# Dahan-Wang/Rethinking-Flow-and-Diffusion-Bridge-Models-for-Speech-Enhancement

Hardware: NVIDIA B200
Metric: enhanced audio-sec/sec (5-step SB bridge, ncsnpp_v2) (higher is better)
Workload: dtype fp16

## Files before the change

### rethinking-flow-and-diffusion-bridge-models-for-speech-enhancement_b200/csrc/conv_igemm.cu

```cuda
#include <cuda.h>
#include <mutex>
#include <type_traits>
#include "common.cuh"
#include "tc05.cuh"

namespace fdbm {
int make_act_tile_map(CUtensorMap* map, const op_t* ptr, int B, int T, int F, int C, int box_f, int box_t);
namespace {

using namespace tc05;

constexpr int MT = 2;
constexpr int TILE_T = 16, TILE_F = 8;
constexpr int HALO_T = TILE_T + 2, HALO_F = TILE_F + 2;
constexpr int A_TILE_BYTES = HALO_T * HALO_F * 128;
constexpr int A_TILE_STRIDE = 23552;
constexpr int A_STAGES = 3;
constexpr int B_STAGES = 3;
constexpr int BN = 128;
constexpr int B_TILE_BYTES = BN * 128;
constexpr int A_SBO = HALO_F * 128;
constexpr int NUM_THREADS = 512;
constexpr int EPI_GROUPS = 2;
constexpr int MAX_SEG = 3;
constexpr int MAX_KB = 16;
constexpr int A_TILE1_BYTES = TILE_T * TILE_F * 128;
constexpr int PIPE_REGS = 56, EPI_REGS = 168, XFORM_REGS = 120;
constexpr int STAGE_BYTES = EPI_GROUPS * 4 * 32 * 32 * 4;
constexpr int STAT_SLOTS = 2;
constexpr int STAT_BYTES = EPI_GROUPS * 4 * BN * 8;
constexpr int B_STAGES_NARROW = B_STAGES * B_TILE_BYTES / (16 * 128);
constexpr int SMEM_BYTES = A_STAGES * MT * A_TILE_STRIDE + B_STAGES * B_TILE_BYTES + STAGE_BYTES + STAT_BYTES + 512;

struct SegParams {
  int taps, norm, act, tab_stride;
  int halo;
  const float2* tab;
};

struct ConvParams {
  int B, T, F, Cout;
  int n_seg, n_kb;
  SegParams seg[MAX_SEG];
  uint32_t ksched[MAX_KB];
  int tiles_t, tiles_f, n_mtiles, n_nblocks, n_items;
  uint32_t mg_tiles_t, mg_tiles_f, mg_nblocks;
  int bn;
  int side_ring, n_main, side_gap, n_steps;
  const float* bias;
  const float* bias_b;
  int bias_b_stride;
  const float* residual;
  const op_t* residual_h16;
  float scale;
  float* out_f32;
  op_t* out_h16;
  double* sums;
  float* pyr_out;
  const float* pyr_prev;
  int pyr_C;
  const float* comb_pyr;
  const float* comb_w;
  const float* comb_b;
  int comb_C;
};

struct TileCoord { int b, t0, f0; bool valid; };

__device__ __forceinline__ int fast_div(int n, int d, uint32_t mg) { return d == 1 ? n : static_cast<int>(__umulhi(static_cast<uint32_t>(n), mg)); }
__device__ __forceinline__ int item_tile(const ConvParams& p, int item) { return fast_div(item, p.n_nblocks, p.mg_nblocks); }
__device__ __forceinline__ int item_nblk(const ConvParams& p, int item) { return item - item_tile(p, item) * p.n_nblocks; }

__device__ __forceinline__ TileCoord decode_tile(const ConvParams& p, int mi) {
  TileCoord c;
  c.valid = mi < p.n_mtiles;
  const int rest = fast_div(mi, p.tiles_t, p.mg_tiles_t);
  const int tt = mi - rest * p.tiles_t;
  c.t0 = tt * TILE_T;
  c.b = fast_div(rest, p.tiles_f, p.mg_tiles_f);
  c.f0 = (rest - c.b * p.tiles_f) * TILE_F;
  return c;
}

template <typename F>
__device__ __forceinline__ void walk_steps(const ConvParams& p, F&& f) {
  const int n_side = p.n_kb - p.n_main;
  int sd = 0, cnt = 0;
  for (int m = 0; m < p.n_main; ++m) {
    const int ntaps = p.seg[p.ksched[m] & 15].taps;
    for (int tap = 0; tap < ntaps; ++tap) {
      f(false, m, tap, ntaps);
      if (++cnt == p.side_gap && sd < n_side) { f(true, p.n_main + sd, 0, 1); ++sd; cnt = 0; }
    }
  }
  for (; sd < n_side; ++sd) f(true, p.n_main + sd, 0, 1);
}

template <bool COMB, bool RES16>
__global__ void __launch_bounds__(NUM_THREADS, 1)
conv_igemm_kernel(const __grid_constant__ CUtensorMap map_a0, const __grid_constant__ CUtensorMap map_a1,
                  const __grid_constant__ CUtensorMap map_a2, const __grid_constant__ CUtensorMap map_b,
                  const ConvParams p) {
  extern __shared__ __align__(1024) uint8_t smem_raw[];
  uint8_t* smem = smem_raw;
  if (smem_u32(smem_raw) & 1023u) __trap();
  uint8_t* sA = smem;
  uint8_t* sB = smem + A_STAGES * MT * A_TILE_STRIDE;
  uint8_t* s_stage = sB + B_STAGES * B_TILE_BYTES;
  uint8_t* s_stat = s_stage + STAGE_BYTES;
  uint64_t* bars = reinterpret_cast<uint64_t*>(s_stage + STAGE_BYTES + STAT_BYTES);
  uint64_t* a_full = bars;
  uint64_t* a_empty = a_full + A_STAGES;
  uint64_t* b_full = a_empty + A_STAGES;
  uint64_t* b_empty = b_full + B_STAGES_NARROW;
  uint64_t* acc_full = b_empty + B_STAGES_NARROW;
  const int b_stages = p.bn == 16 ? B_STAGES_NARROW : B_STAGES;
  const int b_stride = p.bn * 128;
  uint64_t* acc_empty = acc_full + 2;
  uint64_t* a_ready = acc_empty + 2;
  uint64_t* side_full = a_ready + A_STAGES;
  uint64_t* side_empty = side_full + 1;
  uint32_t* tmem_slot = reinterpret_cast<uint32_t*>(side_empty + 1);
  static_assert((3 * A_STAGES + 2 * B_STAGES_NARROW + 4 + 2) * 8 + 4 <= 512, "barrier region");
  const int a_stages = p.side_ring ? A_STAGES - 1 : A_STAGES;
  const int n_main = p.side_ring ? p.n_main : p.n_kb;
// ... 14 lines not shown
    if (p.n_seg > 1) tma_prefetch_desc(&map_a1);
    if (p.n_seg > 2) tma_prefetch_desc(&map_a2);
  }
  if (warp == 3) {
    tmem_alloc(tmem_slot, 512);
    tmem_relinquish();
  }
  fence_before_sync();
  __syncthreads();
  fence_after_sync();
  const uint32_t tmem_base = *tmem_slot;
  asm volatile("griddepcontrol.wait;" ::: "memory");
  asm volatile("griddepcontrol.launch_dependents;" ::: "memory");

  if (warp < 4) {
  reg_dec<PIPE_REGS>();
  if (warp == 0) {
    if (lane == 0) {
      uint32_t stage = 0, phase = 0;
      for (int item = blockIdx.x; item < p.n_items; item += gridDim.x) {
        const int ct = item_tile(p, item);
        TileCoord tc[MT];
        int n_valid = 0;
        for (int j = 0; j < MT; ++j) { tc[j] = decode_tile(p, ct * MT + j); n_valid += tc[j].valid; }
        for (int i = 0; i < n_main; ++i) {
          const uint32_t e = p.ksched[i];
          const int sgi = e & 15, c0 = ((e >> 4) & 0xFFF) * 64;
          const int halo = p.seg[sgi].halo;
          mbar_wait_relaxed<256>(a_empty + stage, phase ^ 1);
          mbar_expect_tx(a_full + stage, n_valid * (halo ? A_TILE_BYTES : A_TILE1_BYTES));
          const CUtensorMap* map = sgi == 0 ? &map_a0 : (sgi == 1 ? &map_a1 : &map_a2);
          for (int j = 0; j < MT; ++j) {
            if (!tc[j].valid) continue;
            tma_load_4d(sA + (stage * MT + j) * A_TILE_STRIDE, map, a_full + stage, c0, tc[j].f0 - halo, tc[j].t0 - halo,
                        tc[j].b);
          }
          if (++stage == a_stages) { stage = 0; phase ^= 1; }
        }
      }
    }
  } else if (warp == 3) {
    if (lane == 0 && p.side_ring) {
      uint32_t phase = 0;
      for (int item = blockIdx.x; item < p.n_items; item += gridDim.x) {
        const int ct = item_tile(p, item);
        TileCoord tc[MT];
        int n_valid = 0;
        for (int j = 0; j < MT; ++j) { tc[j] = decode_tile(p, ct * MT + j); n_valid += tc[j].valid; }
        for (int i = n_main; i < n_kb; ++i) {
          const uint32_t e = p.ksched[i];
          const int sgi = e & 15, c0 = ((e >> 4) & 0xFFF) * 64;
          mbar_wait_relaxed<128>(side_empty, phase ^ 1);
          mbar_expect_tx(side_full, n_valid * A_TILE1_BYTES);
          const CUtensorMap* map = sgi == 0 ? &map_a0 : (sgi == 1 ? &map_a1 : &map_a2);
          for (int j = 0; j < MT; ++j) {
            if (!tc[j].valid) continue;
            tma_load_4d(sA + ((A_STAGES - 1) * MT + j) * A_TILE_STRIDE, map, side_full, c0, tc[j].f0, tc[j].t0, tc[j].b);
          }
          phase ^= 1;
        }
      }
    }
  } else if (warp == 1) {
    if (lane == 0) {
      uint32_t stage = 0, phase = 0;
      for (int item = blockIdx.x; item < p.n_items; item += gridDim.x) {
        const int n0 = item_nblk(p, item) * BN;
        if (p.side_ring) {
          walk_steps(p, [&](bool, int idx, int tap, int) {
            const int kt = static_cast<int>(p.ksched[idx] >> 16) + tap;
            mbar_wait_relaxed<128>(b_empty + stage, phase ^ 1);
            mbar_expect_tx(b_full + stage, b_stride);
            tma_load_2d(sB + stage * b_stride, &map_b, b_full + stage, 0, kt * p.Cout + n0);
            if (++stage == b_stages) { stage = 0; phase ^= 1; }
          });
          continue;
        }
        for (int i = 0; i < n_kb; ++i) {
          const uint32_t e = p.ksched[i];
          const int ntaps = p.seg[e & 15].taps;
          int kt = e >> 16;
          for (int tap = 0; tap < ntaps; ++tap, ++kt) {
            mbar_wait_relaxed<128>(b_empty + stage, phase ^ 1);
            mbar_expect_tx(b_full + stage, b_stride);
            tma_load_2d(sB + stage * b_stride, &map_b, b_full + stage, 0, kt * p.Cout + n0);
            if (++stage == b_stages) { stage = 0; phase ^= 1; }
          }
        }
      }
    }
  } else if (warp == 2) {
    const uint32_t idesc = make_idesc_f16(128, p.bn, kOperandIsBf16);
    const uint64_t a_hi9 = make_desc_sw128(0, A_SBO) & 0xFFFFFFFF00000000ull;
    const uint64_t a_hi1 = make_desc_sw128(0, TILE_F * 128) & 0xFFFFFFFF00000000ull;
    const uint64_t b_hi = make_desc_sw128(0, 1024) & 0xFFFFFFFF00000000ull;
    const uint32_t lo_const = 1u << 16;
    const uint32_t sA_lo = (smem_u32(sA) & 0x3FFFF) >> 4, sB_lo = (smem_u32(sB) & 0x3FFFF) >> 4;
    uint32_t sa = 0, pa = 0, sb = 0, pb = 0, as = 0, pacc = 0, ps = 0;
    for (int item = blockIdx.x; item < p.n_items; item += gridDim.x) {
      const int ct = item_tile(p, item);
      const bool valid1 = (ct * MT + 1) < p.n_mtiles;
      mbar_wait(acc_empty + as, pacc ^ 1);
      fence_after_sync();
      uint32_t accumulate = 0;
      const uint32_t d0 = tmem_base + (as * MT) * BN, d1 = d0 + BN;
      if (p.side_ring) {
        int step = 0;
        walk_steps(p, [&](bool side, int idx, int tap, int ntaps) {
          const SegParams& sg = p.seg[p.ksched[idx] & 15];
          uint32_t a_base0, a_off = 0;
          if (side) {
            mbar_wait(side_full, ps);
            fence_after_sync();
            a_base0 = sA_lo + (((A_STAGES - 1) * MT) * A_TILE_STRIDE >> 4);
          } else {
            if (tap == 0) {
              mbar_wait(sg.norm ? a_ready + sa : a_full + sa, pa);
              fence_after_sync();
            }
            a_base0 = sA_lo + ((sa * MT) * A_TILE_STRIDE >> 4);
            const int df = ntaps == 9 ? tap / 3 : sg.halo, dt = ntaps == 9 ? tap - 3 * (tap / 3) : sg.halo;
            a_off = ((dt * HALO_F + df) * 128) >> 4;
          }
          const uint64_t a_hi = sg.halo ? a_hi9 : a_hi1;
          mbar_wait(b_full + sb, pb);
          fence_after_sync();
          const uint32_t b_lo = (sB_lo + (sb * b_stride >> 4)) | lo_const;
          const uint32_t a_lo0 = (a_base0 + a_off) | lo_const, a_lo1 = (a_base0 + (A_TILE_STRIDE >> 4) + a_off) | lo_const;
          const bool last_tap = tap == ntaps - 1;
          if (elect_one()) {
#pragma unroll
            for (int k = 0; k < 4; ++k)
              mma_f16(d0, a_hi | (a_lo0 + 2 * k), b_hi | (b_lo + 2 * k), idesc, k == 0 ? accumulate : 1u);
            if (valid1) {
#pragma unroll
              for (int k = 0; k < 4; ++k)
                mma_f16(d1, a_hi | (a_lo1 + 2 * k), b_hi | (b_lo + 2 * k), idesc, k == 0 ? accumulate : 1u);
            }
            mma_commit(b_empty + sb);
            if (side) mma_commit(side_empty);
            else if (last_tap) mma_commit(a_empty + sa);
            if (step == p.n_steps - 1) mma_commit(acc_full + as);
          }
          __syncwarp();
          accumulate = 1;
          ++step;
          if (++sb == b_stages) { sb = 0; pb ^= 1; }
          if (side) ps ^= 1;
          else if (last_tap && ++sa == a_stages) { sa = 0; pa ^= 1; }
        });
        if (++as == 2) { as = 0; pacc ^= 1; }
        continue;
      }
      for (int i = 0; i < n_kb; ++i) {
        const SegParams& sg = p.seg[p.ksched[i] & 15];
        const int ntaps = sg.taps;
        const uint64_t a_hi = sg.halo ? a_hi9 : a_hi1;
        mbar_wait(sg.norm ? a_ready + sa : a_full + sa, pa);
        fence_after_sync();
        const uint32_t a_base0 = sA_lo + ((sa * MT) * A_TILE_STRIDE >> 4), a_base1 = a_base0 + (A_TILE_STRIDE >> 4);
        int df = ntaps == 9 ? 0 : sg.halo, dt = df;
        for (int tap = 0; tap < ntaps; ++tap) {
          mbar_wait(b_full + sb, pb);
          fence_after_sync();
          const uint32_t a_off = ((dt * HALO_F + df) * 128) >> 4;
          const uint32_t b_lo = (sB_lo + (sb * b_stride >> 4)) | lo_const;
          const uint32_t a_lo0 = (a_base0 + a_off) | lo_const, a_lo1 = (a_base1 + a_off) | lo_const;
          if (elect_one()) {
#pragma unroll
            for (int k = 0; k < 4; ++k)
              mma_f16(d0, a_hi | (a_lo0 + 2 * k), b_hi | (b_lo + 2 * k), idesc, k == 0 ? accumulate : 1u);
            if (valid1) {
#pragma unroll
              for (int k = 0; k < 4; ++k)
                mma_f16(d1, a_hi | (a_lo1 + 2 * k), b_hi | (b_lo + 2 * k), idesc, k == 0 ? accumulate : 1u);
            }
            mma_commit(b_empty + sb);
            if (tap == ntaps - 1) mma_commit(a_empty + sa);
            if (tap == ntaps - 1 && i == n_kb - 1) mma_commit(acc_full + as);
          }
          __syncwarp();
          accumulate = 1;
          if (++dt == 3) { dt = 0; ++df; }
          if (++sb == b_stages) { sb = 0; pb ^= 1; }
        }
        if (++sa == A_STAGES) { sa = 0; pa ^= 1; }
      }
      if (++as == 2) { as = 0; pacc ^= 1; }
    }
  }
  } else if (warp >= 8 && warp < 12) {
    reg_dec<XFORM_REGS>();
    const int tt = threadIdx.x - 256;
    const int g = tt & 7, p_lane = tt >> 3;
    uint32_t stage = 0, phase = 0;
    const bool any_norm = (p.seg[0].norm | p.seg[1].norm | p.seg[2].norm) != 0;
    for (int item = blockIdx.x; any_norm && item < p.n_items; item += gridDim.x) {
      const int ct = item_tile(p, item);
      TileCoord tc[MT];
      for (int j = 0; j < MT; ++j) tc[j] = decode_tile(p, ct * MT + j);
      for (int i = 0; i < n_main; ++i) {
        const uint32_t e = p.ksched[i];
        const SegParams& sg = p.seg[e & 15];
        float2 sc[MT][4], sh[MT][4];
        if (sg.norm) {
          const int c0 = ((e >> 4) & 0xFFF) * 64 + g * 8;
          const float pre = sg.act ? 0.5f : 1.0f;
#pragma unroll
          for (int j = 0; j < MT; ++j) {
            const float4* tp = reinterpret_cast<const float4*>(sg.tab + static_cast<int64_t>(tc[j].valid ? tc[j].b : 0) * sg.tab_stride + c0);
#pragma unroll
            for (int u = 0; u < 4; ++u) {
              const float4 e = __ldg(tp + u);
              sc[j][u] = make_float2(pre * e.x, pre * e.z); sh[j][u] = make_float2(pre * e.y, pre * e.w);
            }
          }
        }
        mbar_wait_relaxed(a_full + stage, phase);
        if (sg.norm) {
#pragma unroll
          for (int j = 0; j < MT; ++j) {
            if (!tc[j].valid) continue;
            const int r_lo = tc[j].t0 == 0 ? 1 : 0, r_hi = min(HALO_T, p.T - tc[j].t0 + 1);
            const int c_lo = tc[j].f0 == 0 ? 1 : 0, c_hi = min(HALO_F, p.F - tc[j].f0 + 1);
            const bool interior = r_lo == 0 && c_lo == 0 && r_hi == HALO_T && c_hi == HALO_F;
            uint8_t* tile = sA + (stage * MT + j) * A_TILE_STRIDE;
            constexpr int N_PASS = (HALO_T * HALO_F + 63) / 64;
            auto xform = [&](uint4& rawv, auto act_tag) {
              constexpr bool ACT = decltype(act_tag)::value;
              op2_t* h2 = reinterpret_cast<op2_t*>(&rawv);
#pragma unroll
              for (int w = 0; w < 4; ++w) {
                const float2 y = __ffma2_rn(op22f2(h2[w]), sc[j][w], sh[j][w]);
                if (ACT) {
                  const op2_t h = f2op2(y.x, y.y);
                  h2[w] = __hfma2(h, op2_tanh(h), h);
                } else {
                  h2[w] = f2op2(y.x, y.y);
                }
              }
            };
            auto run_interior = [&](auto act_tag) {
              uint8_t* base = tile + p_lane * 128 + ((g ^ (p_lane & 7)) << 4);
#pragma unroll
              for (int pass = 0; pass < N_PASS; ++pass) {
                uint4 raw[4];
#pragma unroll
                for (int u = 0; u < 4; ++u) {
                  const int i = pass * 4 + u;
                  if (i < 11 || p_lane < 4) raw[u] = *reinterpret_cast<uint4*>(base + i * 2048);
                }
#pragma unroll
                for (int u = 0; u < 4; ++u) xform(raw[u], act_tag);
#pragma unroll
                for (int u = 0; u < 4; ++u) {
                  const int i = pass * 4 + u;
                  if (i < 11 || p_lane < 4) *reinterpret_cast<uint4*>(base + i * 2048) = raw[u];
                }
              }
            };
            auto run_border = [&](auto act_tag) {
#pragma unroll 1
              for (int pass = 0; pass < N_PASS; ++pass) {
                uint4 raw[4];
                uint4* slot[4];
                bool on[4];
#pragma unroll
                for (int u = 0; u < 4; ++u) {
                  const int px = p_lane + 16 * (pass * 4 + u);
                  const int hr = px / HALO_F, hc = px - hr * HALO_F;
                  on[u] = px < HALO_T * HALO_F && hr >= r_lo && hr < r_hi && hc >= c_lo && hc < c_hi;
                  slot[u] = reinterpret_cast<uint4*>(tile + px * 128 + ((g ^ (px & 7)) << 4));
                  raw[u] = on[u] ? *slot[u] : make_uint4(0u, 0u, 0u, 0u);
                }
#pragma unroll
                for (int u = 0; u < 4; ++u) xform(raw[u], act_tag);
#pragma unroll
                for (int u = 0; u < 4; ++u)
                  if (on[u]) *slot[u] = raw[u];
              }
            };
            if (interior) { if (sg.act) run_interior(std::true_type{}); else run_interior(std::false_type{}); }
            else { if (sg.act) run_border(std::true_type{}); else run_border(std::false_type{}); }
          }
          fence_proxy_async();
        }
        mbar_arrive(a_ready + stage);
        if (++stage == a_stages) { stage = 0; phase ^= 1; }
      }
    }
  } else {
    reg_inc<EPI_REGS>();
    const int q = warp & 3;
    const int eg = warp >= 12 ? 1 : 0;
    float4* stage = reinterpret_cast<float4*>(s_stage) + (eg * 4 + q) * (32 * 8);
    const int cc = lane & 7;
    const int rsub = lane >> 3;
    const int et = (threadIdx.x & 127);
    uint32_t as = 0, pacc = 0;
    const bool do_stats = p.sums != nullptr;
    float2* wstat = reinterpret_cast<float2*>(s_stat) + eg * 4 * BN;
    double acc_s[STAT_SLOTS], acc_q[STAT_SLOTS];
#pragma unroll
    for (int u = 0; u < STAT_SLOTS; ++u) { acc_s[u] = 0.0; acc_q[u] = 0.0; }
    int stat_b = -1;
    auto flush_stats = [&]() {
#pragma unroll
      for (int u = 0; u < STAT_SLOTS; ++u) {
        if (u < p.n_nblocks) {
          if (et < p.bn) {
            double* dst = p.sums + (static_cast<int64_t>(stat_b) * p.Cout + u * BN + et) * 2;
            atomicAdd(dst, acc_s[u]);
            atomicAdd(dst + 1, acc_q[u]);
          }
        }
        acc_s[u] = 0.0; acc_q[u] = 0.0;
      }
    };
    for (int item = blockIdx.x; item < p.n_items; item += gridDim.x) {
      const int ct = item_tile(p, item);
      const int nblk = item - ct * p.n_nblocks;
      const int n0 = nblk * BN;
      mbar_wait_relaxed(acc_full + as, pacc);
      fence_after_sync();
      for (int j = eg; j <= eg; ++j) {
        const TileCoord tc = decode_tile(p, ct * MT + j);
        if (!tc.valid) continue;
        if (do_stats && stat_b != tc.b) {
          if (stat_b >= 0) flush_stats();
          stat_b = tc.b;
        }
        if (p.pyr_out) {
          uint32_t v[32];
          tmem_ld_32x32(tmem_base + ((q * 32u) << 16) + (as * MT + j) * BN, v);
          tmem_ld_wait();
          const int m = q * 32 + lane;
          const int t = tc.t0 + (m >> 3), f = tc.f0 + (m & 7);
          if (t < p.T && f < p.F) {
            float o[4];
#pragma unroll
            for (int c = 0; c < 4; ++c) o[c] = c < p.pyr_C ? __uint_as_float(v[c]) + __ldg(p.bias + c) : 0.f;
            if (p.pyr_prev) {
              const int Tp = p.T >> 1, Fp = p.F >> 1;
              const int t_a = (t & 1) ? (t >> 1) : (t >> 1) - 1, f_a = (f & 1) ? (f >> 1) : (f >> 1) - 1;
              const float wt_a = (t & 1) ? 0.75f : 0.25f, wf_a = (f & 1) ? 0.75f : 0.25f;
              const float* pb = p.pyr_prev + static_cast<int64_t>(tc.b) * Tp * Fp * p.pyr_C;
              if (p.pyr_C == 4) {
                float4 tap[4];
                float wg[4];
// ... 33 lines not shown
            if (p.pyr_C == 4) *reinterpret_cast<float4*>(dst) = make_float4(o[0], o[1], o[2], o[3]);
            else for (int c = 0; c < p.pyr_C; ++c) dst[c] = o[c];
          }
          continue;
        }
        const bool full = tc.t0 + TILE_T <= p.T && tc.f0 + TILE_F <= p.F;
        const int64_t tile_base = ((static_cast<int64_t>(tc.b) * p.T + tc.t0) * p.F + tc.f0) * p.Cout + n0 + cc * 4;
        const int roff0 = ((q * 4) * p.F + rsub) * p.Cout, roff_t = p.F * p.Cout, roff_f = 4 * p.Cout;
        auto roff = [&](int it) { return roff0 + (it >> 1) * roff_t + (it & 1) * roff_f; };
        uint32_t okmask = 0;
#pragma unroll
        for (int it = 0; it < 8; ++it) {
          const int m = q * 32 + it * 4 + rsub;
          const bool ok = tc.t0 + (m >> 3) < p.T && tc.f0 + (m & 7) < p.F;
          okmask |= ok ? (1u << it) : 0u;
        }
        const float* res_p = !RES16 && p.residual ? p.residual + tile_base : nullptr;
        const op_t* res16_p = RES16 ? p.residual_h16 + tile_base : nullptr;
        float* of_p = p.out_f32 ? p.out_f32 + tile_base : nullptr;
        op_t* oh_p = p.out_h16 ? p.out_h16 + tile_base : nullptr;
        if (RES16 || res_p) {
          const int nitem = item + gridDim.x;
          const int nct = item_tile(p, nitem);
          const int nmi = nitem < p.n_items ? nct * MT + j : p.n_mtiles;
          const int nblk_n = nitem - nct * p.n_nblocks;
          const TileCoord nt = decode_tile(p, nmi);
          const int t = nt.t0 + (et >> 3), f = nt.f0 + (et & 7);
          if (nt.valid && t < p.T && f < p.F) {
            const int64_t po = ((static_cast<int64_t>(nt.b) * p.T + t) * p.F + f) * p.Cout + nblk_n * BN;
            if (RES16) {
#pragma unroll
              for (int u = 0; u < 2; ++u) asm volatile("prefetch.global.L2 [%0];" ::"l"(p.residual_h16 + po + u * 64));
            } else {
#pragma unroll
              for (int u = 0; u < 4; ++u) asm volatile("prefetch.global.L2 [%0];" ::"l"(p.residual + po + u * 32));
            }
          }
        }
        const float2 sc2 = make_float2(p.scale, p.scale);
        const float* bias_p = p.bias + n0 + cc * 4;
        const float* biasb_p = p.bias_b ? p.bias_b + static_cast<int64_t>(tc.b) * p.bias_b_stride + n0 + cc * 4 : nullptr;
        float4 bv = __ldg(reinterpret_cast<const float4*>(bias_p));
        float4 bvb = biasb_p ? __ldg(reinterpret_cast<const float4*>(biasb_p)) : make_float4(0.f, 0.f, 0.f, 0.f);
        float4 res[8];
        uint2 res16_buf[2][8];
        auto load_res16 = [&](int ch) {
          uint2 (&dst)[8] = res16_buf[ch & 1];
          if (full) {
#pragma unroll
            for (int it = 0; it < 8; ++it) dst[it] = __ldg(reinterpret_cast<const uint2*>(res16_p + roff(it) + ch * 32));
          } else {
// ... 199 lines not shown
  for (int u = 0; u < kPackChunk / 256; ++u) {
    const int64_t i = i0 + u * 256 + threadIdx.x;
    if (i < d.total) { if (d.kind == 0) pack_fwd_element(d, i); else pack_dgrad_element(d, i); }
  }
}

typedef CUresult (*EncodeFn)(CUtensorMap*, CUtensorMapDataType, cuuint32_t, void*, const cuuint64_t*, const cuuint64_t*,
                             const cuuint32_t*, const cuuint32_t*, CUtensorMapInterleave, CUtensorMapSwizzle,
                             CUtensorMapL2promotion, CUtensorMapFloatOOBfill);

EncodeFn get_encode() {
  static EncodeFn fn = nullptr;
  static std::once_flag once;
  std::call_once(once, [] {
    void* p = nullptr;
    cudaDriverEntryPointQueryResult q;
    if (cudaGetDriverEntryPoint("cuTensorMapEncodeTiled", &p, cudaEnableDefault, &q) == cudaSuccess &&
        q == cudaDriverEntryPointSuccess)
      fn = reinterpret_cast<EncodeFn>(p);
  });
  return fn;
}

int make_act_map(CUtensorMap* map, const op_t* ptr, int B, int T, int F, int C) {
  return make_act_tile_map(map, ptr, B, T, F, C, HALO_F, HALO_T);
}

int make_weight_map(CUtensorMap* map, const op_t* ptr, int64_t rows, int bn) {
  EncodeFn enc = get_encode();
  if (!enc) { set_error("cuTensorMapEncodeTiled entry point not available"); return FDBM_ECUDA; }
  cuuint64_t dims[2] = {64, (cuuint64_t)rows};
  cuuint64_t strides[1] = {128};
  cuuint32_t box[2] = {64, (cuuint32_t)bn};
  cuuint32_t es[2] = {1, 1};
  CUresult r = enc(map, (kOperandIsBf16 ? CU_TENSOR_MAP_DATA_TYPE_BFLOAT16 : CU_TENSOR_MAP_DATA_TYPE_FLOAT16), 2, const_cast<op_t*>(ptr), dims, strides, box, es,
                   CU_TENSOR_MAP_INTERLEAVE_NONE, CU_TENSOR_MAP_SWIZZLE_128B, CU_TENSOR_MAP_L2_PROMOTION_L2_256B,
                   CU_TENSOR_MAP_FLOAT_OOB_FILL_NONE);
  if (r != CUDA_SUCCESS) { set_error("cuTensorMapEncodeTiled(weights, %lld rows) failed: %d", (long long)rows, (int)r); return FDBM_ECUDA; }
  return FDBM_OK;
}

}

int make_act_tile_map(CUtensorMap* map, const op_t* ptr, int B, int T, int F, int C, int box_f, int box_t) {
  EncodeFn enc = get_encode();
  if (!enc) { set_error("cuTensorMapEncodeTiled entry point not available"); return FDBM_ECUDA; }
  cuuint64_t dims[4] = {(cuuint64_t)C, (cuuint64_t)F, (cuuint64_t)T, (cuuint64_t)B};
  cuuint64_t strides[3] = {(cuuint64_t)C * 2, (cuuint64_t)C * 2 * F, (cuuint64_t)C * 2 * F * T};
  cuuint32_t box[4] = {64, (cuuint32_t)box_f, (cuuint32_t)box_t, 1};
  cuuint32_t es[4] = {1, 1, 1, 1};
// ... 47 lines not shown
  pack_one_kernel<<<static_cast<int>(std::min<int64_t>(ceil_div64(d.total, 256), 4096)), 256, 0, s>>>(d);
  FDBM_LAUNCH_CHECK();
  return FDBM_OK;
}

int launch_pack_conv_weights_dgrad(const float* w, int Cout, int Cin, int ksize, op_t* wpack, cudaStream_t s, int Cin_total, int ci_off) {
  FDBM_REQUIRE(Cout % 64 == 0 && Cin % 64 == 0 && (ksize == 1 || ksize == 3 || ksize == -1),
               "pack_conv_weights_dgrad: channels must be multiples of 64, ksize 1, 3 or -1 (NIN)");
  const PackDesc d = pack_desc_dgrad(w, Cout, Cin, ksize, wpack, Cin_total, ci_off);
  pack_one_kernel<<<static_cast<int>(std::min<int64_t>(ceil_div64(d.total, 256), 4096)), 256, 0, s>>>(d);
  FDBM_LAUNCH_CHECK();
  return FDBM_OK;
}

int launch_conv_igemm(const ConvArgs& a, cudaStream_t s) {
  FDBM_REQUIRE(a.n_seg >= 1 && a.n_seg <= MAX_SEG, "conv_igemm: 1..%d K segments", MAX_SEG);
  const int bn = a.narrow_n ? 16 : (a.Cout == 64 ? 64 : BN);
  FDBM_REQUIRE(a.Cout % bn == 0 && (!a.narrow_n || (a.Cout == 16 && a.pyr_out)), "conv_igemm: Cout must be a multiple of %d (got %d)", bn, a.Cout);
  FDBM_REQUIRE(a.out_f32 || a.out_h16 || a.pyr_out, "conv_igemm: no output");
  FDBM_REQUIRE(!a.pyr_out || (a.pyr_C >= 1 && a.pyr_C <= 4 && a.Cout == bn && !a.sums), "conv_igemm: bad pyramid epilogue arguments");
  FDBM_REQUIRE(!a.pyr_prev || (a.T % 2 == 0 && a.F % 2 == 0), "conv_igemm: pyramid level with odd size");
  static PerDeviceOnce attr_once;
  if (attr_once.first(current_device())) {
    FDBM_CUDA(cudaFuncSetAttribute(conv_igemm_kernel<false, false>, cudaFuncAttributeMaxDynamicSharedMemorySize, SMEM_BYTES));
    FDBM_CUDA(cudaFuncSetAttribute(conv_igemm_kernel<false, true>, cudaFuncAttributeMaxDynamicSharedMemorySize, SMEM_BYTES));
    FDBM_CUDA(cudaFuncSetAttribute(conv_igemm_kernel<true, false>, cudaFuncAttributeMaxDynamicSharedMemorySize, SMEM_BYTES));
  }
  FDBM_REQUIRE(!a.comb_pyr || (a.comb_w && a.comb_b && a.comb_C >= 1 && a.comb_C <= 4 && !a.pyr_out), "conv_igemm: bad Combine epilogue arguments");
  CUtensorMap map_a[MAX_SEG], map_b;
  ConvParams p;
  p.B = a.B; p.T = a.T; p.F = a.F; p.Cout = a.Cout;
  p.n_seg = a.n_seg;
  int kb = 0, n_kt = 0;
  for (int i = 0; i < MAX_SEG; ++i) {
    if (i < a.n_seg) {
      const ConvSeg& sg = a.seg[i];
      FDBM_REQUIRE(sg.in && sg.C > 0 && sg.C % 64 == 0 && (sg.taps == 9 || sg.taps == 1),
                   "conv_igemm: segment %d needs a tensor, C %% 64 == 0 and 9 or 1 taps (C=%d, taps=%d)", i, sg.C, sg.taps);
      const int halo = sg.taps == 9 || sg.norm_tab != nullptr;
      if (int rc = halo ? make_act_map(&map_a[i], sg.in, a.B, a.T, a.F, sg.C)
                        : make_act_tile_map(&map_a[i], sg.in, a.B, a.T, a.F, sg.C, TILE_F, TILE_T)) return rc;
      p.seg[i].halo = halo;
      kb += sg.C / 64; p.seg[i].taps = sg.taps;
      p.seg[i].norm = sg.norm_tab != nullptr; p.seg[i].act = sg.act; p.seg[i].tab = sg.norm_tab;
      p.seg[i].tab_stride = sg.tab_stride;
      n_kt += (sg.C / 64) * sg.taps;
    } else {
      map_a[i] = map_a[0];
      p.seg[i] = SegParams{1, 0, 0, 0, 0, nullptr};
    }
  }
  p.n_kb = kb;
  FDBM_REQUIRE(kb <= MAX_KB, "conv_igemm: at most %d K-blocks (got %d)", MAX_KB, kb);
  {
    uint32_t nine[MAX_KB], one[MAX_KB];
    int n9 = 0, n1 = 0, kt = 0;
    for (int i = 0; i < a.n_seg; ++i)
      for (int cb = 0; cb < a.seg[i].C / 64; ++cb) {
        const uint32_t e = static_cast<uint32_t>(i) | (static_cast<uint32_t>(cb) << 4) | (static_cast<uint32_t>(kt) << 16);
        if (a.seg[i].taps == 9) nine[n9++] = e; else one[n1++] = e;
        kt += a.seg[i].taps;
      }
    int n = 0;
    for (int i = 0; i < n9; ++i) p.ksched[n++] = nine[i];
    for (int i = 0; i < n1; ++i) p.ksched[n++] = one[i];
    for (; n < MAX_KB; ++n) p.ksched[n] = 0;
    bool side_ok = n1 > 0 && n9 > 0;
    for (int i = 0; i < a.n_seg; ++i) side_ok = side_ok && (a.seg[i].taps == 9 || !p.seg[i].halo);
    p.side_ring = side_ok ? 1 : 0;
    p.n_main = p.side_ring ? n9 : kb;
    p.side_gap = p.side_ring ? std::max(3, ceil_div(9 * n9, n1)) : 0;
    p.n_steps = n_kt;
  }
  if (int rc = make_weight_map(&map_b, a.wpack, static_cast<int64_t>(n_kt) * a.Cout, bn)) return rc;
  p.bn = bn;
  p.tiles_t = ceil_div(a.T, TILE_T); p.tiles_f = ceil_div(a.F, TILE_F);
  p.n_mtiles = a.B * p.tiles_t * p.tiles_f;
  p.n_nblocks = a.Cout / bn;
  p.n_items = ceil_div(p.n_mtiles, MT) * p.n_nblocks;
  {
    auto magic = [](int d) { return static_cast<uint32_t>((0x100000000ull + d - 1) / static_cast<uint64_t>(d)); };
    p.mg_tiles_t = magic(p.tiles_t); p.mg_tiles_f = magic(p.tiles_f); p.mg_nblocks = magic(p.n_nblocks);
    const int64_t dmax = std::max(std::max(p.tiles_t, p.tiles_f), p.n_nblocks);
    FDBM_REQUIRE((2 * (static_cast<int64_t>(p.n_items) + num_sms()) + 2) * dmax < 0x100000000ll, "conv_igemm: %d items exceed the range of the index arithmetic", p.n_items);
  }
  p.bias = a.bias; p.bias_b = a.bias_b; p.bias_b_stride = a.bias_b_stride; p.residual = a.residual; p.scale = a.scale;
  p.residual_h16 = a.residual_h16;
  FDBM_REQUIRE(!(a.residual && a.residual_h16) && !(a.residual_h16 && (a.comb_pyr || a.pyr_out)), "conv_igemm: bad residual arguments");
  p.out_f32 = a.out_f32; p.out_h16 = a.out_h16; p.sums = a.sums;
  p.pyr_out = a.pyr_out; p.pyr_prev = a.pyr_prev; p.pyr_C = a.pyr_C;
  p.comb_pyr = a.comb_pyr; p.comb_w = a.comb_w; p.comb_b = a.comb_b; p.comb_C = a.comb_C;
  if (a.sums) {
    FDBM_REQUIRE(p.n_nblocks <= STAT_SLOTS, "conv_igemm: channel sums support Cout <= %d", STAT_SLOTS * BN);
    if (!a.sums_prezeroed) FDBM_CUDA(cudaMemsetAsync(a.sums, 0, sizeof(double) * 2 * a.B * a.Cout, s));
  }
  const int grid = std::min(p.n_items, num_sms());
  cudaLaunchConfig_t cfg = {};
  cfg.gridDim = dim3(grid); cfg.blockDim = dim3(NUM_THREADS); cfg.dynamicSmemBytes = SMEM_BYTES; cfg.stream = s;
  cudaLaunchAttribute attr[1];
  attr[0].id = cudaLaunchAttributeProgrammaticStreamSerialization;
  attr[0].val.programmaticStreamSerializationAllowed = 1;
  cfg.attrs = attr; cfg.numAttrs = pdl_enabled() && a.B <= pdl_batch_limit() ? 1 : 0;
  if (a.comb_pyr) FDBM_CUDA(cudaLaunchKernelEx(&cfg, conv_igemm_kernel<true, false>, map_a[0], map_a[1], map_a[2], map_b, p));
  else if (a.residual_h16) FDBM_CUDA(cudaLaunchKernelEx(&cfg, conv_igemm_kernel<false, true>, map_a[0], map_a[1], map_a[2], map_b, p));
  else FDBM_CUDA(cudaLaunchKernelEx(&cfg, conv_igemm_kernel<false, false>, map_a[0], map_a[1], map_a[2], map_b, p));
  FDBM_LAUNCH_CHECK();
  return FDBM_OK;
}

}

using namespace fdbm;

extern "C" int fdbm_pack_conv_weights(const float* w1, int C1, int ksize, const float* w2, int C2, int Cout,
                                      void* wpack, int64_t* bytes, void* stream) {
  const int k = ksize == -1 ? 1 : ksize;
  if (bytes) *bytes = ksize == -2 ? static_cast<int64_t>(Cout) * 64 * 2 : conv_wpack_bytes(C1, k, C2, Cout);
  if (!wpack) return FDBM_OK;
  if (int rc = require_sm100()) return rc;
  FDBM_REQUIRE(w1 && ((C2 == 0) == (w2 == nullptr)), "fdbm_pack_conv_weights: null pointer");
  FDBM_REQUIRE(ksize != -2 || (C1 >= 1 && 9 * C1 <= 64 && C2 == 0), "fdbm_pack_conv_weights: ksize -2 needs 9 * C1 <= 64 and no second operand");
  return launch_pack_conv_weights(w1, C1, ksize, w2, C2, Cout, Cout, 0, reinterpret_cast<op_t*>(wpack),
                                  as_stream(stream));
}

extern "C" int fdbm_pack_conv_weights_dgrad(const float* w, int Cout, int Cin, int ksize, void* wpack, int64_t* bytes,
                                            void* stream) {
  const int k = ksize == -1 ? 1 : ksize;
// ... 47 lines not shown
```

Before: 1330.

## Load two F-adjacent conv tiles as one shared halo box when F divisible by 16

When F is a multiple of 16, the two M-tiles of a work item are made horizontally adjacent in F. They are fetched with a single 18x18 TMA box instead of two separate 18x10 haloed boxes, so the overlapping halo columns are shared. This cuts the A-operand bytes loaded and normalized per stage, and the MMA descriptors use the wider pitch. It adds FPAIR kernel template variants and refactors the norm/activation transform into a helper, at the cost of more instantiations and different tile scheduling.

```diff
diff --git a/rethinking-flow-and-diffusion-bridge-models-for-speech-enhancement_b200/csrc/conv_igemm.cu b/rethinking-flow-and-diffusion-bridge-models-for-speech-enhancement_b200/csrc/conv_igemm.cu
--- a/rethinking-flow-and-diffusion-bridge-models-for-speech-enhancement_b200/csrc/conv_igemm.cu
+++ b/rethinking-flow-and-diffusion-bridge-models-for-speech-enhancement_b200/csrc/conv_igemm.cu
@@ -13,18 +13,17 @@
 constexpr int MT = 2;
 constexpr int TILE_T = 16, TILE_F = 8;
 constexpr int HALO_T = TILE_T + 2, HALO_F = TILE_F + 2;
-constexpr int A_TILE_BYTES = HALO_T * HALO_F * 128;
+constexpr int PAIR_F = 2 * TILE_F, PAIR_HALO_F = PAIR_F + 2;
 constexpr int A_TILE_STRIDE = 23552;
+constexpr int A_PAIR_STRIDE = 41984;
 constexpr int A_STAGES = 3;
 constexpr int B_STAGES = 3;
 constexpr int BN = 128;
 constexpr int B_TILE_BYTES = BN * 128;
-constexpr int A_SBO = HALO_F * 128;
 constexpr int NUM_THREADS = 512;
 constexpr int EPI_GROUPS = 2;
 constexpr int MAX_SEG = 3;
 constexpr int MAX_KB = 16;
-constexpr int A_TILE1_BYTES = TILE_T * TILE_F * 128;
 constexpr int PIPE_REGS = 56, EPI_REGS = 168, XFORM_REGS = 120;
 constexpr int STAGE_BYTES = EPI_GROUPS * 4 * 32 * 32 * 4;
 constexpr int STAT_SLOTS = 2;
@@ -43,7 +42,7 @@
   int n_seg, n_kb;
   SegParams seg[MAX_SEG];
   uint32_t ksched[MAX_KB];
-  int tiles_t, tiles_f, n_mtiles, n_nblocks, n_items;
+  int tiles_t, tiles_f, n_units, n_nblocks, n_items;
   uint32_t mg_tiles_t, mg_tiles_f, mg_nblocks;
   int bn;
   int side_ring, n_main, side_gap, n_steps;
@@ -71,14 +70,26 @@
 __device__ __forceinline__ int item_tile(const ConvParams& p, int item) { return fast_div(item, p.n_nblocks, p.mg_nblocks); }
 __device__ __forceinline__ int item_nblk(const ConvParams& p, int item) { return item - item_tile(p, item) * p.n_nblocks; }
 
-__device__ __forceinline__ TileCoord decode_tile(const ConvParams& p, int mi) {
+template <bool FPAIR>
+struct Geom {
+  static constexpr int BOXES = FPAIR ? 1 : MT;
+  static constexpr int BOX_F = FPAIR ? PAIR_HALO_F : HALO_F;
+  static constexpr int STAGE = FPAIR ? A_PAIR_STRIDE : MT * A_TILE_STRIDE;
+  static constexpr int TILE1_OFF = FPAIR ? TILE_F * 128 : A_TILE_STRIDE;
+  static constexpr int UNIT_F = FPAIR ? PAIR_F : TILE_F;
+  static constexpr int UNITS = FPAIR ? 1 : MT;
+};
+
+template <bool FPAIR>
+__device__ __forceinline__ TileCoord decode_tile(const ConvParams& p, int ct, int j) {
   TileCoord c;
-  c.valid = mi < p.n_mtiles;
-  const int rest = fast_div(mi, p.tiles_t, p.mg_tiles_t);
-  const int tt = mi - rest * p.tiles_t;
+  const int u = FPAIR ? ct : ct * MT + j;
+  c.valid = u < p.n_units;
+  const int rest = fast_div(u, p.tiles_t, p.mg_tiles_t);
+  const int tt = u - rest * p.tiles_t;
   c.t0 = tt * TILE_T;
   c.b = fast_div(rest, p.tiles_f, p.mg_tiles_f);
-  c.f0 = (rest - c.b * p.tiles_f) * TILE_F;
+  c.f0 = (rest - c.b * p.tiles_f) * Geom<FPAIR>::UNIT_F + (FPAIR ? j * TILE_F : 0);
   return c;
 }
 
@@ -96,11 +107,77 @@
   for (; sd < n_side; ++sd) f(true, p.n_main + sd, 0, 1);
 }
 
-template <bool COMB, bool RES16>
+template <int BOX_F, bool ACT, bool BORDER>
+__device__ __forceinline__ void xform_run(uint8_t* box, int g, int p_lane, const float2 (&sc)[4], const float2 (&sh)[4],
+                                          int r_lo, int r_hi, int c_lo, int c_hi) {
+  constexpr int N_FULL = HALO_T * BOX_F / 16, REM = HALO_T * BOX_F % 16;
+  constexpr int N_PASS = (N_FULL + (REM ? 1 : 0) + 3) / 4;
+  uint8_t* base = box + p_lane * 128 + ((g ^ (p_lane & 7)) << 4);
+  uint32_t off = 0;
+  if (BORDER) {
+#pragma unroll 1
+    for (int i = 0; i <= N_FULL; ++i) {
+      const int px = p_lane + 16 * i, hr = px / BOX_F, hc = px - hr * BOX_F;
+      off |= (hr < r_lo || hr >= r_hi || hc < c_lo || hc >= c_hi) ? 1u << i : 0u;
+    }
+  }
+  auto xform = [&](uint4& rawv) {
+    op2_t* h2 = reinterpret_cast<op2_t*>(&rawv);
+#pragma unroll
+    for (int w = 0; w < 4; ++w) {
+      const float2 y = __ffma2_rn(op22f2(h2[w]), sc[w], sh[w]);
+      if (ACT) {
+        const op2_t h = f2op2(y.x, y.y);
+        h2[w] = __hfma2(h, op2_tanh(h), h);
+      } else {
+        h2[w] = f2op2(y.x, y.y);
+      }
+    }
+  };
+#pragma unroll
+  for (int pass = 0; pass < N_PASS; ++pass) {
+    uint4 raw[4];
+#pragma unroll
+    for (int u = 0; u < 4; ++u) {
+      const int i = pass * 4 + u;
+      if (i < N_FULL || (i == N_FULL && p_lane < REM)) raw[u] = *reinterpret_cast<uint4*>(base + i * 2048);
+    }
+#pragma unroll
+    for (int u = 0; u < 4; ++u)
+      if (pass * 4 + u <= N_FULL) xform(raw[u]);
+#pragma unroll
+    for (int u = 0; u < 4; ++u) {
+      const int i = pass * 4 + u;
+      if (i < N_FULL || (i == N_FULL && p_lane < REM)) {
+        if (BORDER && ((off >> i) & 1u)) raw[u] = make_uint4(0u, 0u, 0u, 0u);
+        *reinterpret_cast<uint4*>(base + i * 2048) = raw[u];
+      }
+    }
+  }
+}
+
+template <int BOX_F>
+__device__ __forceinline__ void xform_box(const ConvParams& p, const TileCoord& tc, uint8_t* box, int g, int p_lane, int act,
+                                          const float2 (&sc)[4], const float2 (&sh)[4]) {
+  if (!tc.valid) return;
+  const int r_lo = tc.t0 == 0 ? 1 : 0, r_hi = min(HALO_T, p.T - tc.t0 + 1);
+  const int c_lo = tc.f0 == 0 ? 1 : 0, c_hi = min(BOX_F, p.F - tc.f0 + 1);
+  const bool interior = r_lo == 0 && c_lo == 0 && r_hi == HALO_T && c_hi == BOX_F;
+  if (interior) {
+    if (act) xform_run<BOX_F, true, false>(box, g, p_lane, sc, sh, r_lo, r_hi, c_lo, c_hi);
+    else xform_run<BOX_F, false, false>(box, g, p_lane, sc, sh, r_lo, r_hi, c_lo, c_hi);
+  } else {
+    if (act) xform_run<BOX_F, true, true>(box, g, p_lane, sc, sh, r_lo, r_hi, c_lo, c_hi);
+    else xform_run<BOX_F, false, true>(box, g, p_lane, sc, sh, r_lo, r_hi, c_lo, c_hi);
+  }
+}
+
+template <bool COMB, bool RES16, bool FPAIR>
 __global__ void __launch_bounds__(NUM_THREADS, 1)
 conv_igemm_kernel(const __grid_constant__ CUtensorMap map_a0, const __grid_constant__ CUtensorMap map_a1,
                   const __grid_constant__ CUtensorMap map_a2, const __grid_constant__ CUtensorMap map_b,
                   const ConvParams p) {
+  using G = Geom<FPAIR>;
   extern __shared__ __align__(1024) uint8_t smem_raw[];
   uint8_t* smem = smem_raw;
   if (smem_u32(smem_raw) & 1023u) __trap();
@@ -161,17 +238,19 @@
         const int ct = item_tile(p, item);
         TileCoord tc[MT];
         int n_valid = 0;
-        for (int j = 0; j < MT; ++j) { tc[j] = decode_tile(p, ct * MT + j); n_valid += tc[j].valid; }
+#pragma unroll
+        for (int j = 0; j < MT; ++j) { tc[j] = decode_tile<FPAIR>(p, ct, j); n_valid += j < G::BOXES && tc[j].valid; }
         for (int i = 0; i < n_main; ++i) {
           const uint32_t e = p.ksched[i];
           const int sgi = e & 15, c0 = ((e >> 4) & 0xFFF) * 64;
           const int halo = p.seg[sgi].halo;
           mbar_wait_relaxed<256>(a_empty + stage, phase ^ 1);
-          mbar_expect_tx(a_full + stage, n_valid * (halo ? A_TILE_BYTES : A_TILE1_BYTES));
+          mbar_expect_tx(a_full + stage, n_valid * (halo ? HALO_T * G::BOX_F : TILE_T * (G::BOX_F - 2)) * 128);
           const CUtensorMap* map = sgi == 0 ? &map_a0 : (sgi == 1 ? &map_a1 : &map_a2);
+#pragma unroll
           for (int j = 0; j < MT; ++j) {
-            if (!tc[j].valid) continue;
-            tma_load_4d(sA + (stage * MT + j) * A_TILE_STRIDE, map, a_full + stage, c0, tc[j].f0 - halo, tc[j].t0 - halo,
+            if (j >= G::BOXES || !tc[j].valid) continue;
+            tma_load_4d(sA + stage * G::STAGE + j * G::TILE1_OFF, map, a_full + stage, c0, tc[j].f0 - halo, tc[j].t0 - halo,
                         tc[j].b);
           }
           if (++stage == a_stages) { stage = 0; phase ^= 1; }
@@ -185,16 +264,18 @@
         const int ct = item_tile(p, item);
         TileCoord tc[MT];
         int n_valid = 0;
-        for (int j = 0; j < MT; ++j) { tc[j] = decode_tile(p, ct * MT + j); n_valid += tc[j].valid; }
+#pragma unroll
+        for (int j = 0; j < MT; ++j) { tc[j] = decode_tile<FPAIR>(p, ct, j); n_valid += j < G::BOXES && tc[j].valid; }
         for (int i = n_main; i < n_kb; ++i) {
           const uint32_t e = p.ksched[i];
           const int sgi = e & 15, c0 = ((e >> 4) & 0xFFF) * 64;
           mbar_wait_relaxed<128>(side_empty, phase ^ 1);
-          mbar_expect_tx(side_full, n_valid * A_TILE1_BYTES);
+          mbar_expect_tx(side_full, n_valid * TILE_T * (G::BOX_F - 2) * 128);
           const CUtensorMap* map = sgi == 0 ? &map_a0 : (sgi == 1 ? &map_a1 : &map_a2);
+#pragma unroll
           for (int j = 0; j < MT; ++j) {
-            if (!tc[j].valid) continue;
-            tma_load_4d(sA + ((A_STAGES - 1) * MT + j) * A_TILE_STRIDE, map, side_full, c0, tc[j].f0, tc[j].t0, tc[j].b);
+            if (j >= G::BOXES || !tc[j].valid) continue;
+            tma_load_4d(sA + (A_STAGES - 1) * G::STAGE + j * G::TILE1_OFF, map, side_full, c0, tc[j].f0, tc[j].t0, tc[j].b);
           }
           phase ^= 1;
         }
@@ -230,15 +311,16 @@
     }
   } else if (warp == 2) {
     const uint32_t idesc = make_idesc_f16(128, p.bn, kOperandIsBf16);
-    const uint64_t a_hi9 = make_desc_sw128(0, A_SBO) & 0xFFFFFFFF00000000ull;
-    const uint64_t a_hi1 = make_desc_sw128(0, TILE_F * 128) & 0xFFFFFFFF00000000ull;
+    const uint64_t a_hi9 = make_desc_sw128(0, G::BOX_F * 128) & 0xFFFFFFFF00000000ull;
+    const uint64_t a_hi1 = make_desc_sw128(0, (G::BOX_F - 2) * 128) & 0xFFFFFFFF00000000ull;
     const uint64_t b_hi = make_desc_sw128(0, 1024) & 0xFFFFFFFF00000000ull;
     const uint32_t lo_const = 1u << 16;
     const uint32_t sA_lo = (smem_u32(sA) & 0x3FFFF) >> 4, sB_lo = (smem_u32(sB) & 0x3FFFF) >> 4;
+    const uint32_t a_stage16 = G::STAGE >> 4, tile1_16 = G::TILE1_OFF >> 4, pitch16 = G::BOX_F * 8;
     uint32_t sa = 0, pa = 0, sb = 0, pb = 0, as = 0, pacc = 0, ps = 0;
     for (int item = blockIdx.x; item < p.n_items; item += gridDim.x) {
       const int ct = item_tile(p, item);
-      const bool valid1 = (ct * MT + 1) < p.n_mtiles;
+      const bool valid1 = decode_tile<FPAIR>(p, ct, 1).valid;
       mbar_wait(acc_empty + as, pacc ^ 1);
       fence_after_sync();
       uint32_t accumulate = 0;
@@ -251,21 +333,21 @@
           if (side) {
             mbar_wait(side_full, ps);
             fence_after_sync();
-            a_base0 = sA_lo + (((A_STAGES - 1) * MT) * A_TILE_STRIDE >> 4);
+            a_base0 = sA_lo + (A_STAGES - 1) * a_stage16;
           } else {
             if (tap == 0) {
               mbar_wait(sg.norm ? a_ready + sa : a_full + sa, pa);
               fence_after_sync();
             }
-            a_base0 = sA_lo + ((sa * MT) * A_TILE_STRIDE >> 4);
+            a_base0 = sA_lo + sa * a_stage16;
             const int df = ntaps == 9 ? tap / 3 : sg.halo, dt = ntaps == 9 ? tap - 3 * (tap / 3) : sg.halo;
-            a_off = ((dt * HALO_F + df) * 128) >> 4;
+            a_off = dt * pitch16 + df * 8;
           }
           const uint64_t a_hi = sg.halo ? a_hi9 : a_hi1;
           mbar_wait(b_full + sb, pb);
           fence_after_sync();
           const uint32_t b_lo = (sB_lo + (sb * b_stride >> 4)) | lo_const;
-          const uint32_t a_lo0 = (a_base0 + a_off) | lo_const, a_lo1 = (a_base0 + (A_TILE_STRIDE >> 4) + a_off) | lo_const;
+          const uint32_t a_lo0 = (a_base0 + a_off) | lo_const, a_lo1 = (a_base0 + tile1_16 + a_off) | lo_const;
           const bool last_tap = tap == ntaps - 1;
           if (elect_one()) {
 #pragma unroll
@@ -297,12 +379,12 @@
         const uint64_t a_hi = sg.halo ? a_hi9 : a_hi1;
         mbar_wait(sg.norm ? a_ready + sa : a_full + sa, pa);
         fence_after_sync();
-        const uint32_t a_base0 = sA_lo + ((sa * MT) * A_TILE_STRIDE >> 4), a_base1 = a_base0 + (A_TILE_STRIDE >> 4);
+        const uint32_t a_base0 = sA_lo + sa * a_stage16, a_base1 = a_base0 + tile1_16;
         int df = ntaps == 9 ? 0 : sg.halo, dt = df;
         for (int tap = 0; tap < ntaps; ++tap) {
           mbar_wait(b_full + sb, pb);
           fence_after_sync();
-          const uint32_t a_off = ((dt * HALO_F + df) * 128) >> 4;
+          const uint32_t a_off = dt * pitch16 + df * 8;
           const uint32_t b_lo = (sB_lo + (sb * b_stride >> 4)) | lo_const;
           const uint32_t a_lo0 = (a_base0 + a_off) | lo_const, a_lo1 = (a_base1 + a_off) | lo_const;
           if (elect_one()) {
@@ -337,7 +419,7 @@
     for (int item = blockIdx.x; any_norm && item < p.n_items; item += gridDim.x) {
       const int ct = item_tile(p, item);
       TileCoord tc[MT];
-      for (int j = 0; j < MT; ++j) tc[j] = decode_tile(p, ct * MT + j);
+      for (int j = 0; j < MT; ++j) tc[j] = decode_tile<FPAIR>(p, ct, j);
       for (int i = 0; i < n_main; ++i) {
         const uint32_t e = p.ksched[i];
         const SegParams& sg = p.seg[e & 15];
@@ -347,6 +429,7 @@
           const float pre = sg.act ? 0.5f : 1.0f;
 #pragma unroll
           for (int j = 0; j < MT; ++j) {
+            if (j >= G::BOXES) break;
             const float4* tp = reinterpret_cast<const float4*>(sg.tab + static_cast<int64_t>(tc[j].valid ? tc[j].b : 0) * sg.tab_stride + c0);
 #pragma unroll
             for (int u = 0; u < 4; ++u) {
@@ -357,70 +440,12 @@
         }
         mbar_wait_relaxed(a_full + stage, phase);
         if (sg.norm) {
-#pragma unroll
-          for (int j = 0; j < MT; ++j) {
-            if (!tc[j].valid) continue;
-            const int r_lo = tc[j].t0 == 0 ? 1 : 0, r_hi = min(HALO_T, p.T - tc[j].t0 + 1);
-            const int c_lo = tc[j].f0 == 0 ? 1 : 0, c_hi = min(HALO_F, p.F - tc[j].f0 + 1);
-            const bool interior = r_lo == 0 && c_lo == 0 && r_hi == HALO_T && c_hi == HALO_F;
-            uint8_t* tile = sA + (stage * MT + j) * A_TILE_STRIDE;
-            constexpr int N_PASS = (HALO_T * HALO_F + 63) / 64;
-            auto xform = [&](uint4& rawv, auto act_tag) {
-              constexpr bool ACT = decltype(act_tag)::value;
-              op2_t* h2 = reinterpret_cast<op2_t*>(&rawv);
-#pragma unroll
-              for (int w = 0; w < 4; ++w) {
-                const float2 y = __ffma2_rn(op22f2(h2[w]), sc[j][w], sh[j][w]);
-                if (ACT) {
-                  const op2_t h = f2op2(y.x, y.y);
-                  h2[w] = __hfma2(h, op2_tanh(h), h);
-                } else {
-                  h2[w] = f2op2(y.x, y.y);
-                }
-              }
-            };
-            auto run_interior = [&](auto act_tag) {
-              uint8_t* base = tile + p_lane * 128 + ((g ^ (p_lane & 7)) << 4);
-#pragma unroll
-              for (int pass = 0; pass < N_PASS; ++pass) {
-                uint4 raw[4];
-#pragma unroll
-                for (int u = 0; u < 4; ++u) {
-                  const int i = pass * 4 + u;
-                  if (i < 11 || p_lane < 4) raw[u] = *reinterpret_cast<uint4*>(base + i * 2048);
-                }
-#pragma unroll
-                for (int u = 0; u < 4; ++u) xform(raw[u], act_tag);
-#pragma unroll
-                for (int u = 0; u < 4; ++u) {
-                  const int i = pass * 4 + u;
-                  if (i < 11 || p_lane < 4) *reinterpret_cast<uint4*>(base + i * 2048) = raw[u];
-                }
-              }
-            };
-            auto run_border = [&](auto act_tag) {
-#pragma unroll 1
-              for (int pass = 0; pass < N_PASS; ++pass) {
-                uint4 raw[4];
-                uint4* slot[4];
-                bool on[4];
-#pragma unroll
-                for (int u = 0; u < 4; ++u) {
-                  const int px = p_lane + 16 * (pass * 4 + u);
-                  const int hr = px / HALO_F, hc = px - hr * HALO_F;
-                  on[u] = px < HALO_T * HALO_F && hr >= r_lo && hr < r_hi && hc >= c_lo && hc < c_hi;
-                  slot[u] = reinterpret_cast<uint4*>(tile + px * 128 + ((g ^ (px & 7)) << 4));
-                  raw[u] = on[u] ? *slot[u] : make_uint4(0u, 0u, 0u, 0u);
-                }
-#pragma unroll
-                for (int u = 0; u < 4; ++u) xform(raw[u], act_tag);
-#pragma unroll
-                for (int u = 0; u < 4; ++u)
-                  if (on[u]) *slot[u] = raw[u];
-              }
-            };
-            if (interior) { if (sg.act) run_interior(std::true_type{}); else run_interior(std::false_type{}); }
-            else { if (sg.act) run_border(std::true_type{}); else run_border(std::false_type{}); }
+          uint8_t* box0 = sA + stage * G::STAGE;
+          if constexpr (FPAIR) {
+            xform_box<PAIR_HALO_F>(p, tc[0], box0, g, p_lane, sg.act, sc[0], sh[0]);
+          } else {
+            xform_box<HALO_F>(p, tc[0], box0, g, p_lane, sg.act, sc[0], sh[0]);
+            xform_box<HALO_F>(p, tc[1], box0 + A_TILE_STRIDE, g, p_lane, sg.act, sc[1], sh[1]);
           }
           fence_proxy_async();
         }
@@ -463,7 +488,7 @@
       mbar_wait_relaxed(acc_full + as, pacc);
       fence_after_sync();
       for (int j = eg; j <= eg; ++j) {
-        const TileCoord tc = decode_tile(p, ct * MT + j);
+        const TileCoord tc = decode_tile<FPAIR>(p, ct, j);
         if (!tc.valid) continue;
         if (do_stats && stat_b != tc.b) {
           if (stat_b >= 0) flush_stats();
@@ -543,11 +568,10 @@
         if (RES16 || res_p) {
           const int nitem = item + gridDim.x;
           const int nct = item_tile(p, nitem);
-          const int nmi = nitem < p.n_items ? nct * MT + j : p.n_mtiles;
           const int nblk_n = nitem - nct * p.n_nblocks;
-          const TileCoord nt = decode_tile(p, nmi);
+          const TileCoord nt = decode_tile<FPAIR>(p, nct, j);
           const int t = nt.t0 + (et >> 3), f = nt.f0 + (et & 7);
-          if (nt.valid && t < p.T && f < p.F) {
+          if (nitem < p.n_items && nt.valid && t < p.T && f < p.F) {
             const int64_t po = ((static_cast<int64_t>(nt.b) * p.T + t) * p.F + f) * p.Cout + nblk_n * BN;
             if (RES16) {
 #pragma unroll
@@ -793,10 +817,6 @@
   return fn;
 }
 
-int make_act_map(CUtensorMap* map, const op_t* ptr, int B, int T, int F, int C) {
-  return make_act_tile_map(map, ptr, B, T, F, C, HALO_F, HALO_T);
-}
-
 int make_weight_map(CUtensorMap* map, const op_t* ptr, int64_t rows, int bn) {
   EncodeFn enc = get_encode();
   if (!enc) { set_error("cuTensorMapEncodeTiled entry point not available"); return FDBM_ECUDA; }
@@ -890,15 +910,18 @@
   FDBM_REQUIRE(!a.pyr_prev || (a.T % 2 == 0 && a.F % 2 == 0), "conv_igemm: pyramid level with odd size");
   static PerDeviceOnce attr_once;
   if (attr_once.first(current_device())) {
-    FDBM_CUDA(cudaFuncSetAttribute(conv_igemm_kernel<false, false>, cudaFuncAttributeMaxDynamicSharedMemorySize, SMEM_BYTES));
-    FDBM_CUDA(cudaFuncSetAttribute(conv_igemm_kernel<false, true>, cudaFuncAttributeMaxDynamicSharedMemorySize, SMEM_BYTES));
-    FDBM_CUDA(cudaFuncSetAttribute(conv_igemm_kernel<true, false>, cudaFuncAttributeMaxDynamicSharedMemorySize, SMEM_BYTES));
+    for (auto k : {conv_igemm_kernel<false, false, false>, conv_igemm_kernel<false, true, false>, conv_igemm_kernel<true, false, false>,
+                   conv_igemm_kernel<false, false, true>, conv_igemm_kernel<false, true, true>, conv_igemm_kernel<true, false, true>})
+      FDBM_CUDA(cudaFuncSetAttribute(k, cudaFuncAttributeMaxDynamicSharedMemorySize, SMEM_BYTES));
   }
   FDBM_REQUIRE(!a.comb_pyr || (a.comb_w && a.comb_b && a.comb_C >= 1 && a.comb_C <= 4 && !a.pyr_out), "conv_igemm: bad Combine epilogue arguments");
   CUtensorMap map_a[MAX_SEG], map_b;
   ConvParams p;
   p.B = a.B; p.T = a.T; p.F = a.F; p.Cout = a.Cout;
   p.n_seg = a.n_seg;
+  const bool fpair = a.F % PAIR_F == 0;
+  const int box_f = fpair ? Geom<true>::BOX_F : Geom<false>::BOX_F, unit_f = fpair ? Geom<true>::UNIT_F : Geom<false>::UNIT_F;
+  const int units_per_item = fpair ? Geom<true>::UNITS : Geom<false>::UNITS;
   int kb = 0, n_kt = 0;
   for (int i = 0; i < MAX_SEG; ++i) {
     if (i < a.n_seg) {
@@ -906,8 +929,8 @@
       FDBM_REQUIRE(sg.in && sg.C > 0 && sg.C % 64 == 0 && (sg.taps == 9 || sg.taps == 1),
                    "conv_igemm: segment %d needs a tensor, C %% 64 == 0 and 9 or 1 taps (C=%d, taps=%d)", i, sg.C, sg.taps);
       const int halo = sg.taps == 9 || sg.norm_tab != nullptr;
-      if (int rc = halo ? make_act_map(&map_a[i], sg.in, a.B, a.T, a.F, sg.C)
-                        : make_act_tile_map(&map_a[i], sg.in, a.B, a.T, a.F, sg.C, TILE_F, TILE_T)) return rc;
+      if (int rc = halo ? make_act_tile_map(&map_a[i], sg.in, a.B, a.T, a.F, sg.C, box_f, HALO_T)
+                        : make_act_tile_map(&map_a[i], sg.in, a.B, a.T, a.F, sg.C, box_f - 2, TILE_T)) return rc;
       p.seg[i].halo = halo;
       kb += sg.C / 64; p.seg[i].taps = sg.taps;
       p.seg[i].norm = sg.norm_tab != nullptr; p.seg[i].act = sg.act; p.seg[i].tab = sg.norm_tab;
@@ -942,10 +965,10 @@
   }
   if (int rc = make_weight_map(&map_b, a.wpack, static_cast<int64_t>(n_kt) * a.Cout, bn)) return rc;
   p.bn = bn;
-  p.tiles_t = ceil_div(a.T, TILE_T); p.tiles_f = ceil_div(a.F, TILE_F);
-  p.n_mtiles = a.B * p.tiles_t * p.tiles_f;
+  p.tiles_t = ceil_div(a.T, TILE_T); p.tiles_f = ceil_div(a.F, unit_f);
+  p.n_units = a.B * p.tiles_t * p.tiles_f;
   p.n_nblocks = a.Cout / bn;
-  p.n_items = ceil_div(p.n_mtiles, MT) * p.n_nblocks;
+  p.n_items = ceil_div(p.n_units, units_per_item) * p.n_nblocks;
   {
     auto magic = [](int d) { return static_cast<uint32_t>((0x100000000ull + d - 1) / static_cast<uint64_t>(d)); };
     p.mg_tiles_t = magic(p.tiles_t); p.mg_tiles_f = magic(p.tiles_f); p.mg_nblocks = magic(p.n_nblocks);
@@ -969,9 +992,11 @@
   attr[0].id = cudaLaunchAttributeProgrammaticStreamSerialization;
   attr[0].val.programmaticStreamSerializationAllowed = 1;
   cfg.attrs = attr; cfg.numAttrs = pdl_enabled() && a.B <= pdl_batch_limit() ? 1 : 0;
-  if (a.comb_pyr) FDBM_CUDA(cudaLaunchKernelEx(&cfg, conv_igemm_kernel<true, false>, map_a[0], map_a[1], map_a[2], map_b, p));
-  else if (a.residual_h16) FDBM_CUDA(cudaLaunchKernelEx(&cfg, conv_igemm_kernel<false, true>, map_a[0], map_a[1], map_a[2], map_b, p));
-  else FDBM_CUDA(cudaLaunchKernelEx(&cfg, conv_igemm_kernel<false, false>, map_a[0], map_a[1], map_a[2], map_b, p));
+  auto kernel = fpair ? (a.comb_pyr ? conv_igemm_kernel<true, false, true>
+                                     : (a.residual_h16 ? conv_igemm_kernel<false, true, true> : conv_igemm_kernel<false, false, true>))
+                      : (a.comb_pyr ? conv_igemm_kernel<true, false, false>
+                                    : (a.residual_h16 ? conv_igemm_kernel<false, true, false> : conv_igemm_kernel<false, false, false>));
+  FDBM_CUDA(cudaLaunchKernelEx(&cfg, kernel, map_a[0], map_a[1], map_a[2], map_b, p));
   FDBM_LAUNCH_CHECK();
   return FDBM_OK;
 }
```

Result: faster. 1349, median of 6 (+1.5%).
